# centreborelli/sat-bundleadjust

Hardware: AMD Instinct MI355X
Metric: LM iters/sec at 200 cams x 1M pts x 10M obs (affine, R+T) (higher is better)
Workload: dtype f64; 1 GPU; C4: 200 cams x 1000000 pts x 9998866 obs, affine, correction R+T, 1 fixed camera, seed 1; obs_per_rank0=9998866

## Files before the change

### sat-bundleadjust_amd/csrc/satba_capi.hip

```cpp
#include <hip/hip_runtime.h>

#include <algorithm>
#include <atomic>
#include <chrono>
#include <cmath>
#include <cstdarg>
#include <cstdio>
#include <cstdlib>
#include <cstring>
#include <new>
#include <string>
#include <thread>
#include <vector>

#include "../../include/satba.h"
#include "satba_chol.h"
#include "satba_kernels.h"
#include "satba_layout.h"
#include "satba_lm.h"
#include "satba_lmdev.h"
#include "satba_outliers.h"
#include "satba_triangulate.h"
#include "satba_tracks.h"
#include "satba_ftracks.h"
#include "satba_match.h"
#include "satba_rpcfit.h"
#include "satba_camapprox.h"
#include "satba_schur.h"
#include "satba_schur_items.h"

#include <dlfcn.h>

namespace {
struct Roctx {
    int (*push)(const char*) = nullptr;
    int (*pop)() = nullptr;
    Roctx() {
        for (const char* name : {"librocprofiler-sdk-roctx.so", "librocprofiler-sdk-roctx.so.1", "libroctx64.so", "libroctx64.so.4"}) {
            if (void* h = dlopen(name, RTLD_LAZY | RTLD_GLOBAL)) {
                push = reinterpret_cast<int (*)(const char*)>(dlsym(h, "roctxRangePushA"));
                pop = reinterpret_cast<int (*)()>(dlsym(h, "roctxRangePop"));
                if (push && pop) return;
                push = nullptr; pop = nullptr;
            }
        }
    }
};
inline const Roctx& roctx() { static const Roctx r; return r; }
struct Range {
    bool on;
    explicit Range(const char* name) : on(roctx().push != nullptr) { if (on) roctx().push(name); }
    ~Range() { if (on) roctx().pop(); }
};
}

using namespace satba;

static thread_local std::string g_err;

static int fail(int code, const char* fmt, ...) {
    char buf[512];
    va_list ap;
    va_start(ap, fmt);
    vsnprintf(buf, sizeof buf, fmt, ap);
    va_end(ap);
    g_err = buf;
    return code;
}

#define HIP_TRY(expr)                                                                                   \
    do {                                                                                                \
        hipError_t e_ = (expr);                                                                         \
        if (e_ != hipSuccess) return fail(SATBA_E_HIP, "%s: %s (%s:%d)", #expr, hipGetErrorString(e_), __FILE__, __LINE__); \
    } while (0)

constexpr int RED_SLOTS = 8, RED_MAX_GRID = 2048, RED_MAX_NV = 4;
struct SchurItems { int2* items = nullptr; SchurItem* desc = nullptr; int n_blocks = 0; };
static_assert(sizeof(SchurItemKey) == sizeof(int2) && offsetof(SchurItemKey, pair) == offsetof(int2, x) && offsetof(SchurItemKey, chunk) == offsetof(int2, y), "uploaded as int2");

struct satba_problem {
    int model = 0, M = 0, N = 0, NP = 0, c_p = 0, n_cam_fix = 0, n_pts_fix = 0, rank = 0, world = 1, f32 = 0, device = 0;
    long long K = 0, n_total = 0;
// ... 5 lines not shown
    int deterministic = 0;
    int split_env = -1;
    double *d_fx = nullptr, *d_bbox = nullptr, *d_fxcost = nullptr, *d_fxcost_new = nullptr, *d_fxcost0 = nullptr;
    int *d_fxflag = nullptr, *d_fxe = nullptr;
    bool fxcost_valid = false, fxcost_new_valid = false, fxcost0_valid = false;
    double w_max = 1.0, n_max_cam = 1.0, fx_shrink = 1.0;
    int fx_fallbacks = 0;
    bool scales_by_tail = false;
    bool gh_in_readers = false;
    bool q1_points_unformed = false;
    bool prep_fused = false;
    struct LmDev* d_lm = nullptr;
    struct LmSummary* h_lm = nullptr;
    struct LmSummary* h_lm_dev = nullptr;
    long long lm_ticks_queued = 0;
    hipStream_t own_stream = nullptr;
    double f_scale = 1.0, lead = 1.0;
    hipStream_t stream = nullptr;
    Layout L;
    int unit_weights = 0;
    double *d_cam_static = nullptr, *d_rpc = nullptr;
    double *d_x = nullptr, *d_xnew = nullptr, *d_camc = nullptr, *d_camc_new = nullptr;
    double *d_scale_inv = nullptr, *d_g = nullptr, *d_gh = nullptr, *d_gn = nullptr, *d_q1 = nullptr, *d_wv = nullptr;
    double *d_U = nullptr, *d_gc = nullptr, *d_V = nullptr, *d_PV = nullptr, *d_dc = nullptr, *d_dch = nullptr;
    double2 *d_f = nullptr, *d_ftmp = nullptr;
    bool f_valid = false;
    bool prof_lin = false;
    std::vector<hipEvent_t> prof_ev;
    size_t prof_used = 0;
    double* d_Jpm = nullptr;
    double *d_part = nullptr, *d_part3 = nullptr, *d_pair_part = nullptr;
    SchurItems items_chunked;
    SchurItems items_merged;
    double2* d_W = nullptr;
    SchurItems items_w;
    int lin_grid = 0, cm_chunks = 1, cm_chunks_w = 1;
    double* d_red = nullptr;
    unsigned* d_red_cnt = nullptr;
    double* d_stage = nullptr;
    size_t stage_len = 0;
    int* d_fail = nullptr;
    double* d_dinv = nullptr;
    CholWork chol;
    bool s_scaled = false;
    hipStream_t chol_stream = nullptr;
    hipEvent_t ev_fork = nullptr, ev_join = nullptr;
    int* d_arrive = nullptr;
    int* d_pair_cnt = nullptr;
    int* d_dg_cnt = nullptr;
    long long* d_ts = nullptr;
    int msg_epoch = 0;
    double* msg_packed = nullptr;
    bool beside_last = false;
    bool beside_off = false;
    int beside_clean = 0;
    int beside_retry_after = 64;
    int beside_timeouts = 0;
    double* d_scal = nullptr;
    double* d_keep = nullptr;
    double* d_lam_used = nullptr;
    bool prepared = false;
    double *d_xb_own = nullptr, *d_xb = nullptr;
    long long xb_len = 0;
    double* h_pin = nullptr;
    bool dir_global = false;
    double* d_dir_tab = nullptr;
    void* h_stage = nullptr;
    size_t h_stage_len = 0;
    struct CopyLane { char* pin = nullptr; hipEvent_t ev[2] = {nullptr, nullptr}; };
    CopyLane lanes[8];
    hipStream_t copy_stream = nullptr;
    bool lanes_ready = false;
    double* d_err_keep = nullptr;
    hipEvent_t ev_err = nullptr;
    double* d_x0 = nullptr;
    bool linearized = false, have_step = false;
    double create_ms[8] = {0, 0, 0, 0, 0, 0, 0, 0};
    std::vector<void*> allocs;

    double* payload() const { return d_xb + hdr; }
    RedBuf red(int slot) const { return RedBuf{d_red + (size_t)slot * RED_MAX_NV * RED_MAX_GRID, d_red_cnt + slot}; }
};
struct PhaseCtx {
    const int* gate = nullptr;
    const double *Delta_dev = nullptr, *coef_dev = nullptr, *lam_force_dev = nullptr, *sub_args_dev = nullptr;
    const int* first_dev = nullptr;
    int fuse_prep = -1;
    bool skip_lin_scales = false;
    bool decide1a_in_trial = false;
    bool decide2_in_trial = false;
};
struct FrontCtx {
    int arrive_epoch = 0;
    bool scale_in_finish = false;
    double lam = 0.0;
    const double* lam_dev = nullptr;
};
enum { RB_RES = 0, RB_LIN = 1, RB_PREP = 2, RB_JVP = 3, RB_BS = 4, RB_SUB = 5, RB_TRIAL = 6, RB_MISC = 7 };

template <class T>
static int dev_alloc(satba_problem* p, T** out, size_t count) {
    void* ptr = nullptr;
    HIP_TRY(hipMalloc(&ptr, (count ? count : 1) * sizeof(T)));
    p->allocs.push_back(ptr);
    *out = static_cast<T*>(ptr);
    return 0;
// ... 1321 lines not shown
}

int satba_get_layout(satba_problem* p, int32_t which, int64_t n, void* host_out) {
    if (!p || !host_out) return fail(SATBA_E_ARG, "null argument");
    const int64_t len = satba_layout_len(p, which);
    if (len < 0 || n != len) return fail(SATBA_E_ARG, "layout array %d has %lld entries, caller expects %lld", which, (long long)len, (long long)n);
    const Layout& L = p->L;
    const void* src = nullptr;
    size_t esz = sizeof(int);
    switch (which) {
        case SATBA_LAY_PERM: src = L.perm; break;
        case SATBA_LAY_RANK: src = L.rank; break;
        case SATBA_LAY_PT_CNT: src = L.pt_cnt; break;
        case SATBA_LAY_SLICE_BASE: src = L.slice_base; break;
        case SATBA_LAY_E_CAM: src = L.e_cam; break;
        case SATBA_LAY_OBS_POS: src = L.obs_pos; break;
        case SATBA_LAY_CM_PT: src = L.cm_pt; break;
        case SATBA_LAY_CM_POS: src = L.cm_pos; break;
        case SATBA_LAY_CM_IO: src = L.cm_io; break;
        case SATBA_LAY_IPT_OFS: src = L.ipt_ofs; break;
        case SATBA_LAY_CAM_OFS: src = L.cam_ofs; break;
        case SATBA_LAY_PAIR_OFS: src = L.pair_ofs; esz = sizeof(long long); break;
        case SATBA_LAY_PAIR_PTS: src = L.pair_pts; break;
        case SATBA_LAY_PAIR_PI: src = L.pair_pi; break;
        case SATBA_LAY_PAIR_PJ: src = L.pair_pj; break;
        case SATBA_LAY_PAIR_IJ: src = L.pair_ij; break;
        case SATBA_LAY_W_FIX: src = L.w_fix; break;
        case SATBA_LAY_SC_OFS: src = L.sc_ofs; break;
        case SATBA_LAY_PAIR_REC: src = L.pair_rec; break;
        case SATBA_LAY_PAIR_KK: src = L.pair_kk; break;
        case SATBA_LAY_CM_REC: src = L.cm_rec; break;
        case SATBA_LAY_CM_SC: src = L.cm_sc; break;
        case SATBA_LAY_DG_OFS: src = L.dg_ofs; break;
        default: return fail(SATBA_E_ARG, "unknown layout array %d", which);
    }
    HIP_TRY(hipSetDevice(p->device));
    HIP_TRY(hipStreamSynchronize(p->stream));
    if (len) HIP_TRY(hipMemcpy(host_out, src, esz * (size_t)len, hipMemcpyDeviceToHost));
    return 0;
}

int satba_get_info(const satba_problem* p, double* out, int32_t n) {
    if (!p || !out || n < 16) return fail(SATBA_E_ARG, "bad argument");
    for (int i = 0; i < n; ++i) out[i] = 0.0;
    for (int i = 0; i < 5; ++i) out[i] = p->create_ms[i];
    out[5] = p->L.P; out[6] = (double)p->L.E; out[7] = p->L.C; out[8] = p->unit_weights; out[9] = p->camc_lds; out[10] = p->rpc_lds;
    out[11] = p->cam_sums_lds; out[12] = p->deterministic; out[13] = p->cm_chunks; out[14] = p->lin_grid; out[15] = p->fx_fallbacks;
    if (n > 16) out[16] = (lm_device_loop_ok(p) && lm_device_loop_pays(p)) ? 1.0 : 0.0;
    if (n > 17) out[17] = p->beside_off ? -1.0 : (p->beside_last ? 1.0 : 0.0);
    if (n > 18) out[18] = p->beside_timeouts;
    if (n > 19) out[19] = p->L.wl_ready ? p->L.dg_spc : 0;
    if (n > 20) out[20] = slice_split(p);
    if (n > 21) out[21] = p->lin_rep_shift;
    return 0;
}

int satba_time_kernel(satba_problem* p, int32_t phase, int32_t reps, float* ms_avg) {
    if (!p || !ms_avg || reps <= 0) return fail(SATBA_E_ARG, "bad argument");
    if (phase < 0 || phase > 5) return fail(SATBA_E_ARG, "unknown phase %d", phase);
    if (phase >= 2 && !p->linearized) return fail(SATBA_E_STATE, "time_kernel: linearize first");
    HIP_TRY(hipSetDevice(p->device));
    hipEvent_t e0, e1;
    HIP_TRY(hipEventCreate(&e0));
    HIP_TRY(hipEventCreate(&e1));
    int rc = 0;
    auto once = [&]() -> int {
        switch (phase) {
            case 0: return launch_residual(p, false, p->d_f, p->d_scal);
            case 1: return launch_linearize_kernel(p, PhaseCtx{}, true);
            case 2: return launch_schur_kernel(p, nullptr, FrontCtx{}, schur_route(p, FrontCtx{}));
            case 3: {
                return dense_solve(p, nullptr, p->payload(), p->d_dch);
            }
            case 4: return launch_backsub_kernel(p, nullptr);
            default: return launch_jvp(p, nullptr, 1, p->d_q1, p->d_q1, p->d_scal, true);
        }
    };
    rc = once();
    if (!rc) {
        (void)hipEventRecord(e0, p->stream);
        for (int i = 0; i < reps && !rc; ++i) rc = once();
        (void)hipEventRecord(e1, p->stream);
        (void)hipEventSynchronize(e1);
        float ms = 0.f;
        (void)hipEventElapsedTime(&ms, e0, e1);
        *ms_avg = ms / reps;
    }
    (void)hipEventDestroy(e0);
    (void)hipEventDestroy(e1);
    p->linearized = false; p->have_step = false;
    return rc;
}

#include "satba_outliers_api.inc"
#include "satba_triangulate_api.inc"
#include "satba_rpcfit_api.inc"
#include "satba_camapprox_api.inc"
#include "satba_tracks_api.inc"
#include "satba_ftracks_api.inc"
#include "satba_match_api.inc"

}
```

### sat-bundleadjust_amd/csrc/satba_schur.h

```cpp
#pragma once
#include "satba_kernels.h"

namespace satba {

constexpr int PV_STRIDE = 16;
__device__ inline double schur_lambda(const double* __restrict__ hdr, double Delta, double lam_floor, double* __restrict__ keep, bool write) {
    const double gh_sq = hdr[SATBA_HDR_GH_SQ], jg_sq = hdr[SATBA_HDR_JG_SQ], xs_sq = hdr[SATBA_HDR_XS_SQ];
    if (!(Delta > 0.0)) {
        Delta = sqrt(xs_sq);
        if (Delta == 0.0) Delta = 1.0;
    }
    const double a = 0.5 * jg_sq, b = -gh_sq, ub = Delta / sqrt(gh_sq);
    double best = fmin(0.0, a * ub * ub + b * ub);
    if (a != 0.0) {
        const double ext = -0.5 * b / a;
        if (0.0 < ext && ext < ub) best = fmin(best, a * ext * ext + b * ext);
    }
    double lam = -best / (Delta * Delta);
    if (!(lam >= lam_floor)) lam = lam_floor;
    if (write) {
        keep[SATBA_KEEP_GINF] = fmax(keep[SATBA_KEEP_GINF], hdr[SATBA_HDR_GC_INF]);
        keep[SATBA_KEEP_GH_SQ] = gh_sq; keep[SATBA_KEEP_JG_SQ] = jg_sq; keep[SATBA_KEEP_XS_SQ] = xs_sq;
        keep[SATBA_KEEP_LAM] = lam;
        keep[SATBA_KEEP_DELTA] = Delta;
// ... 792 lines not shown
                    if constexpr (NP == 5) { acc[k++] += y0[r]; acc[k++] += y1[r]; }
                }
                if constexpr (NP == 5) { acc[k++] += e00; acc[k++] += e01; acc[k++] += e11; }
#pragma unroll
                for (int r = 0; r < 3; ++r) acc[k++] -= D[0][r] * b0 + D[1][r] * b1;
                if constexpr (NP == 5) { acc[k++] -= b0; acc[k++] -= b1; }
            } else {
                double Jc[2][NP], Jp[2][3];
                if constexpr (MODEL == RPC) {
                    ObsEval<MODEL, NP, true> e2;
                    e2.load_d(a, lst_sc[posc]);
                    rpc_jac_from_d<NP>(cc, r0.x, r0.y, r1.x, e2.Dr, Jc, Jp);
#pragma unroll
                    for (int k = 0; k < NP; ++k) { Jc[0][k] *= vm; Jc[1][k] *= vm; }
                    ux = uy = sx = sy = 1.0;
                } else {
                    double u, v;
                    project<MODEL, NP, true>(cc, nullptr, r0.x, r0.y, r1.x, false, u, v, Jc, Jp);
                    if (a.sc) { const double2 t = sc_now; ux = vm * t.x * t.x; uy = vm * t.y * t.y; }
                    sx = ux; sy = uy;
                }
                double A[2][3];
#pragma unroll
                for (int r = 0; r < 2; ++r) {
                    A[r][0] = Jp[r][0] * v00 + Jp[r][1] * v01 + Jp[r][2] * v02;
                    A[r][1] = Jp[r][0] * v01 + Jp[r][1] * v11 + Jp[r][2] * v12;
                    A[r][2] = Jp[r][0] * v02 + Jp[r][1] * v12 + Jp[r][2] * v22;
                }
                const double m00 = sx * ux * (A[0][0] * Jp[0][0] + A[0][1] * Jp[0][1] + A[0][2] * Jp[0][2]);
                const double m01 = sx * uy * (A[0][0] * Jp[1][0] + A[0][1] * Jp[1][1] + A[0][2] * Jp[1][2]);
                const double m11 = sy * uy * (A[1][0] * Jp[1][0] + A[1][1] * Jp[1][1] + A[1][2] * Jp[1][2]);
                const double ag0 = sx * (A[0][0] * r4.y + A[0][1] * r5.x + A[0][2] * r5.y);
                const double ag1 = sy * (A[1][0] * r4.y + A[1][1] * r5.x + A[1][2] * r5.y);
                int k = 0;
#pragma unroll
                for (int r = 0; r < NP; ++r) {
                    const double y0 = m00 * Jc[0][r] + m01 * Jc[1][r];
                    const double y1 = m01 * Jc[0][r] + m11 * Jc[1][r];
#pragma unroll
                    for (int q = r; q < NP; ++q) {
                        acc[k] -= Jc[0][q] * y0 + Jc[1][q] * y1;
                        acc[k] += ux * Jc[0][r] * Jc[0][q] + uy * Jc[1][r] * Jc[1][q];
                        ++k;
                    }
                }
#pragma unroll
                for (int r = 0; r < NP; ++r) acc[k++] -= Jc[0][r] * ag0 + Jc[1][r] * ag1;
            }
            __builtin_amdgcn_sched_barrier(0);
        }
    }
}

template <int MODEL, int NP>
__device__ __forceinline__ void schur_diag_body(const ObsArgs& a, const CamMajor& c, const SchurArgs& s, double* __restrict__ part, const int L, const int M,
                                                const int n_chunks, double2* s_coop, double (*s_red)[cam_acc_len(NP)]) {
    constexpr int CU = cam_acc_len(NP);
    int cam = L % M, chunk = L / M;
    if (s.diag_xcd) {
        const int x = L & 7, q = L >> 3;
        cam = q % M; chunk = (q / M) * 8 + x;
    }
    const int b = c.cam_ofs[cam], e = c.cam_ofs[cam + 1];
    const long long len = e - b;
    const int lo = b + (int)(len * chunk / n_chunks);
    const int hi = cam < a.n_cam_fix ? lo : b + (int)(len * (chunk + 1) / n_chunks);
    const int lane = threadIdx.x & 63, wave = threadIdx.x >> 6;
    double acc[CU];
#pragma unroll
    for (int k = 0; k < CU; ++k) acc[k] = 0.0;
    schur_diag_walk<MODEL, NP, LINC_THREADS>(a, s.PV, c.pt, c.io, s.wmode ? 1 : PV_STRIDE / 2, s.wmode ? s.zero_fix : (PV_STRIDE / 2) * a.N, cam, lo, hi,
                                             (int)threadIdx.x, s_coop + wave * (64 * 7), acc);
#pragma unroll
    for (int k = 0; k < CU; ++k) {
        const double t = wave_sum(acc[k]);
        if (lane == 0) s_red[wave][k] = t;
    }
    __syncthreads();
    if (threadIdx.x < CU) {
        double t = 0.0;
        for (int wv = 0; wv < LINC_THREADS / 64; ++wv) t += s_red[wv][threadIdx.x];
        part[((size_t)cam * n_chunks + chunk) * CU + threadIdx.x] = t;
    }
}
template <int MODEL, int NP>
__global__ __launch_bounds__(LINC_THREADS) void k_schur_diag(ObsArgs a, CamMajor c, SchurArgs s, double* __restrict__ part) {
    SATBA_GATE(a.gate);
    __shared__ double2 s_coop[(LINC_THREADS / 64) * 64 * 7];
    __shared__ double s_red[LINC_THREADS / 64][cam_acc_len(NP)];
    schur_diag_body<MODEL, NP>(a, c, s, part, (int)(blockIdx.y * gridDim.x + blockIdx.x), (int)gridDim.x, (int)gridDim.y, s_coop, s_red);
}
static_assert(LINC_THREADS == 256, "k_schur_both: both bodies run 256 threads");
template <int MODEL, int NP, bool UNITW>
__global__ __launch_bounds__(256) SATBA_PAIRS_WAVES_ATTR(MODEL, NP, UNITW) void k_schur_both(ObsArgs a, CamMajor c, SchurArgs s, double* __restrict__ part, double* __restrict__ S,
                                                                                      int n_diag, int n_diag_pad, int M, int n_chunks) {
    SATBA_GATE(a.gate);
    __shared__ double2 s_coop[4 * 64 * 7];
    __shared__ unsigned s_idx[4][3 * 64];
    __shared__ double s_red[4][cam_acc_len(NP)];
    if ((int)blockIdx.x < n_diag_pad) {
        if ((int)blockIdx.x < n_diag) schur_diag_body<MODEL, NP>(a, c, s, part, (int)blockIdx.x, M, n_chunks, s_coop, s_red);
        return;
    }
    schur_pairs_body<MODEL, NP, UNITW>(a, s, S, blockIdx.x - (unsigned)n_diag_pad, s_coop, s_idx);
}

__global__ __launch_bounds__(256) void k_schur_finish(int M, int NP, int n_c, int n_chunks, const double* __restrict__ part, double lam,
                                                      const double* __restrict__ lam_dev, double lead, const double* __restrict__ gc,
                                                      const double* __restrict__ scale_inv, double* __restrict__ S, double* __restrict__ rhs,
                                                      double* __restrict__ xb, int hdr_len, int nb_diag, int red_chunks,
                                                      const int2* __restrict__ pair_ij, const double* __restrict__ pair_part, const int* gate,
                                                      double* __restrict__ rhs_scaled = nullptr, int* __restrict__ clear = nullptr, int n_clear = 0) {
    SATBA_GATE(gate);
    if ((int)blockIdx.x >= nb_diag) {
        const long long n_pairs = (long long)M * (M - 1) / 2;
        const int NB2 = NP * NP;
        const long long idx = (long long)(blockIdx.x - nb_diag) * blockDim.x + threadIdx.x;
        if (idx >= n_pairs * NB2) return;
        const long long pair = idx / NB2;
        const int e = (int)(idx % NB2);
        double t = 0.0;
        int ch = 0;
        for (; ch + 4 <= red_chunks; ch += 4) {
            const double p0 = pair_part[((size_t)ch * n_pairs + pair) * NB2 + e], p1 = pair_part[((size_t)(ch + 1) * n_pairs + pair) * NB2 + e];
            const double p2 = pair_part[((size_t)(ch + 2) * n_pairs + pair) * NB2 + e], p3 = pair_part[((size_t)(ch + 3) * n_pairs + pair) * NB2 + e];
            t += p0; t += p1; t += p2; t += p3;
        }
        for (; ch < red_chunks; ++ch) t += pair_part[((size_t)ch * n_pairs + pair) * NB2 + e];
        const int2 ij = pair_ij[pair];
        const int r = e / NP, q = e % NP;
        if (rhs_scaled) t /= scale_inv[ij.y * NP + q] * scale_inv[ij.x * NP + r];
        S[(size_t)(ij.y * NP + q) + (size_t)(ij.x * NP + r) * n_c] = t;
        return;
    }
    if (lam_dev) lam = *lam_dev;
    const int CU = cam_acc_len(NP);
    const int gid = blockIdx.x * blockDim.x + threadIdx.x, idx = gid >> 3, sub = gid & 7;
    if (gid < hdr_len) xb[gid] = 0.0;
    if (gid < n_clear) clear[gid] = 0;
    if (n_chunks <= 0) return;
    const bool live = idx < M * CU;
    const int cam = live ? idx / CU : 0, k = live ? idx % CU : 0;
    const double t = schur_diag_total<false>(part, cam, n_chunks, CU, k, sub, live);
    if (!live || sub != 0) return;
    schur_diag_store<false>(cam, k, t, NP, n_c, lam, lead, gc, scale_inv, S, rhs, rhs_scaled);
}

}
```

### sat-bundleadjust_amd/csrc/satba_schur_api.inc

```
extern "C++" {
namespace {

int schur_items_build(satba_problem* p, SchurTable kind, SchurItems* t, long long dg_weight) {
    const bool w = kind == SCHUR_ITEMS_WEIGHTED;
    const std::vector<SchurItemKey> table = schur_item_order(kind, p->M, p->L.C, w ? p->L.dg_spc : 0, dg_weight);
    t->n_blocks = (int)(table.size() / 4);
    TRY(dev_alloc(p, &t->items, table.size()));
    HIP_TRY(hipMemcpy(t->items, table.data(), sizeof(int2) * table.size(), hipMemcpyHostToDevice));
    TRY(dev_alloc(p, &t->desc, table.size()));
    hipLaunchKernelGGL(k_schur_item_desc, dim3((unsigned)((table.size() + 255) / 256)), dim3(256), 0, p->stream, (long long)table.size(), t->items,
                       p->L.pair_ij, p->L.pair_ofs, p->L.C, t->desc, w ? p->L.dg_ofs : (const int*)nullptr, w ? p->L.n_dg : 1);
    HIP_TRY(hipGetLastError());
    return 0;
}
bool schur_merge_enough(const satba_problem* p) {
    const char* mg = getenv("SATBA_SCHUR_MERGE");
    return p->L.n_pairs >= 8192 || (mg && atoi(mg) != 0);
}
int schur_item_tables(satba_problem* p) {
    TRY(schur_items_build(p, SCHUR_ITEMS_CHUNKED, &p->items_chunked, 0));
    const char* mg = getenv("SATBA_SCHUR_MERGE");
    if (p->L.C > 1 && schur_merge_enough(p) && !(mg && atoi(mg) == 0)) TRY(schur_items_build(p, SCHUR_ITEMS_MERGED, &p->items_merged, 0));
    return 0;
}

struct SchurRoute {
    bool pairs_run, unit, weighted;
    const SchurItems* items;
    int n_chunks, red_chunks;
    bool dg_in_pairs, cm_rec;
    int dchunks, diag_xcd;
    bool both;
    bool finish_first, finish_direct, finish_scale;
    int finish_dchunks, finish_red_chunks, nb_diag;
    bool beside_ok;
    int wgs, arr_extra;
};

SchurRoute schur_route(const satba_problem* p, const FrontCtx& f) {
    const bool arrive = f.arrive_epoch != 0;
    static const bool one_launch = !(getenv("SATBA_SCHUR_ONE_LAUNCH") && atoi(getenv("SATBA_SCHUR_ONE_LAUNCH")) == 0);
    SchurRoute r;
    r.pairs_run = pairs_run(p); r.unit = unit_run(p); r.weighted = merged_records(p);
    const bool merged = r.pairs_run && r.unit && p->items_merged.desc;
    r.items = merged ? &p->items_merged : (r.weighted ? &p->items_w : &p->items_chunked);
    r.n_chunks = merged ? 1 : p->L.C; r.red_chunks = (r.pairs_run && p->L.C > 1 && !merged) ? p->L.C : 1;
    r.dg_in_pairs = r.weighted && r.pairs_run;
    r.dchunks = r.dg_in_pairs ? p->L.n_dg : (r.weighted ? p->cm_chunks_w : p->cm_chunks);
    r.diag_xcd = (!r.dg_in_pairs && r.dchunks % 8 == 0 && !getenv("SATBA_NO_DIAG_XCD")) ? 1 : 0;
    r.cm_rec = r.weighted && !r.dg_in_pairs;
    r.both = one_launch && !arrive && !r.dg_in_pairs && r.pairs_run;
    r.finish_first = arrive; r.finish_direct = arrive || (r.pairs_run && r.red_chunks == 1);
    r.finish_dchunks = (arrive && r.dg_in_pairs) ? 0 : r.dchunks; r.finish_red_chunks = arrive ? 1 : r.red_chunks;
    r.nb_diag = (int)((std::max<long long>(8ll * p->M * cam_acc_len(p->NP), p->hdr) + 255) / 256);
    r.finish_scale = f.scale_in_finish &&!r.finish_direct && 1 + CH_MAX_STEPS <= r.nb_diag * 256;
    const char* env = getenv("SATBA_CHOL_BESIDE");
    const bool items_ok = r.unit ? r.red_chunks == 1 : (schur_merge_enough(p) && p->model != RPC);
    r.beside_ok = !(env && atoi(env) == 0) && p->world == 1 && items_ok && r.pairs_run && p->n_c == p->M * p->NP && p->n_c > 128 && p->n_c <= 1024 &&
                  p->N > 0 && !p->beside_off;
    r.wgs = r.weighted ? 16 : 32; r.arr_extra = r.weighted ? 1 : 0;
    return r;
}

SchurArgs schur_args(const satba_problem* p, const FrontCtx& f, const SchurRoute& r, double* rhs) {
    SchurArgs s;
    s.PV = reinterpret_cast<const double2*>(p->d_PV);
    s.pair_ofs = p->L.pair_ofs; s.pair_pts = p->L.pair_pts; s.pair_pi = p->L.pair_pi; s.pair_pj = p->L.pair_pj;
    s.pair_ij = p->L.pair_ij; s.pair_part = p->d_pair_part; s.n_chunks = r.n_chunks; s.items = r.items->items; s.desc = r.items->desc; s.diag_xcd = r.diag_xcd;
    if (r.weighted) {
        s.PV = p->d_W; s.wmode = 1; s.zero_fix = p->L.zero_fix; s.n_dg = p->L.n_dg;
        s.pair_rec = p->L.pair_rec; s.pair_kk = p->L.pair_kk; s.cm_rec = p->L.cm_rec; s.cm_sc = p->L.cm_sc; s.dg_part = p->d_part3;
    }
    if (f.arrive_epoch) {
        s.arrive = p->d_arrive; s.arrive_epoch = f.arrive_epoch; s.pair_cnt = p->d_pair_cnt; s.fail = p->d_fail;
        if (r.dg_in_pairs) {
            s.dg_cnt = p->d_dg_cnt; s.dg_lam = f.lam; s.dg_lam_dev = f.lam_dev; s.dg_lead = p->lead; s.dg_gc = p->d_gc;
            s.dg_scale_inv = p->d_scale_inv; s.dg_rhs = rhs;
        }
    }
    return s;
}

template <int MODEL, int NP>
int launch_schur(satba_problem* p, const FrontCtx& f, const SchurRoute& r, const ObsArgs& a, double* S, double* rhs) {
    if (f.arrive_epoch && r.unit && r.red_chunks > 1) return fail(SATBA_E_STATE, "factorisation beside a unit-weight pair kernel with chunk partials");
    const CamMajor cm = cam_major(p, r.cm_rec);
    const SchurArgs s = schur_args(p, f, r, rhs);
    auto finish = [&]() {
        const long long outs = r.finish_red_chunks > 1 ? p->L.n_pairs * NP * NP : 0;
        hipLaunchKernelGGL(k_schur_finish, dim3((unsigned)(r.nb_diag + (outs + 255) / 256)), dim3(256), 0, p->stream, p->M, NP, p->n_c, r.finish_dchunks, p->d_part3,
                           f.lam, f.lam_dev, p->lead, p->d_gc, p->d_scale_inv, S, rhs, p->d_xb, (int)p->hdr, r.nb_diag, r.finish_red_chunks,
                           p->L.pair_ij, p->d_pair_part, a.gate, r.finish_scale ? p->d_dch : (double*)nullptr, r.finish_scale ? p->d_fail : (int*)nullptr,
                           r.finish_scale ? 1 + CH_MAX_STEPS : 0);
        p->s_scaled = r.finish_scale;
    };
    if (!r.dg_in_pairs && !r.both) hipLaunchKernelGGL((k_schur_diag<MODEL, NP>), dim3(p->M, r.dchunks), dim3(LINC_THREADS), 0, p->stream, a, cm, s, p->d_part3);
    if (r.finish_first) finish();
    if (r.pairs_run) {
        const dim3 igrid((unsigned)r.items->n_blocks);
        if (r.both) {
            const int n_diag = p->M * r.dchunks, n_diag_pad = (n_diag + 7) & ~7;
            const dim3 bgrid(igrid.x + (unsigned)n_diag_pad);
            if (r.unit) hipLaunchKernelGGL((k_schur_both<MODEL, NP, true>), bgrid, dim3(256), 0, p->stream, a, cm, s, p->d_part3, S, n_diag, n_diag_pad, p->M, r.dchunks);
            else hipLaunchKernelGGL((k_schur_both<MODEL, NP, false>), bgrid, dim3(256), 0, p->stream, a, cm, s, p->d_part3, S, n_diag, n_diag_pad, p->M, r.dchunks);
        }
        else if (r.unit) hipLaunchKernelGGL((k_schur_pairs<MODEL, NP, true>), igrid, dim3(256), 0, p->stream, a, s, S);
        else hipLaunchKernelGGL((k_schur_pairs<MODEL, NP, false>), igrid, dim3(256), 0, p->stream, a, s, S);
        HIP_TRY(hipGetLastError());
    }
    if (!r.finish_first) finish();
    HIP_TRY(hipGetLastError());
    return 0;
}

int schur_impl(satba_problem* p, const PhaseCtx& c, FrontCtx f, double lam, bool automatic, double Delta, double lam_floor) {
    Range range_("satba:schur");
    if (!p->linearized || (automatic && !p->prepared)) return fail(SATBA_E_STATE, automatic ? "schur_auto before prepare" : "schur before linearize");
    if (automatic) p->prepared = false;
    const SchurRoute r = schur_route(p, f);
    if (p->N > 0) {
        const bool w = r.weighted;
        hipLaunchKernelGGL(k_vinv, dim3((p->N + VINV_THREADS - 1) / VINV_THREADS), dim3(VINV_THREADS), 0, p->stream, p->N, lam, automatic ? p->d_xb : nullptr, Delta, lam_floor,
                           p->d_keep, p->d_V, p->d_scale_inv + p->n_c, p->d_lam_used, p->d_x + p->n_c, p->d_g + p->n_c, w ? reinterpret_cast<double*>(p->d_W) : p->d_PV,
                           p->L.perm, p->n_pts_fix, automatic ? c.Delta_dev : nullptr, automatic ? c.lam_force_dev : nullptr, c.gate,
                           w ? p->L.w_fix : (const int*)nullptr);
    } else if (automatic) {
        hipLaunchKernelGGL(k_lambda, dim3(1), dim3(1), 0, p->stream, p->d_xb, Delta, lam_floor, p->d_keep, c.Delta_dev, c.lam_force_dev, c.gate);
    }
    HIP_TRY(hipGetLastError());
    if (!r.pairs_run) HIP_TRY(hipMemsetAsync(p->d_xb + p->hdr, 0, sizeof(double) * ((size_t)p->n_c * p->n_c + p->n_c), p->stream));
    f.lam = lam; f.lam_dev = automatic ? p->d_keep + SATBA_KEEP_LAM : nullptr;
    return launch_schur_kernel(p, c.gate, f, r);
}

void beside_disable(satba_problem* p) {
    if (p->beside_timeouts > 0) p->beside_retry_after = std::min(p->beside_retry_after * 2, 1 << 20);
    p->beside_off = true; p->beside_clean = 0; ++p->beside_timeouts;
    (void)hipStreamSynchronize(p->chol_stream);
    (void)hipMemsetAsync(p->d_arrive, 0, sizeof(int) * (size_t)(p->M + 2) * SCHUR_ARRIVE_STRIDE, p->stream);
    (void)hipMemsetAsync(p->d_pair_cnt, 0, sizeof(int) * (size_t)std::max<long long>(p->L.n_pairs, 1), p->stream);
    (void)hipMemsetAsync(p->d_dg_cnt, 0, sizeof(int) * (size_t)p->M, p->stream);
}
bool beside_timed_out(satba_problem* p, const double* h) {
    if (!p->beside_last || !(h[SATBA_HDR_CHOL_FAIL] >= SATBA_CHOL_BESIDE_WAIT)) return false;
    beside_disable(p);
    return true;
}
int chol_front_streams(satba_problem* p) {
    if (p->chol_stream) return 0;
    int least = 0, greatest = 0, mine = 0;
    HIP_TRY(hipDeviceGetStreamPriorityRange(&least, &greatest));
    HIP_TRY(hipStreamGetPriority(p->stream, &mine));
    HIP_TRY(hipStreamCreateWithPriority(&p->chol_stream, hipStreamNonBlocking, mine != greatest ? greatest : least));
    HIP_TRY(hipEventCreateWithFlags(&p->ev_fork, hipEventDisableTiming));
    HIP_TRY(hipEventCreateWithFlags(&p->ev_join, hipEventDisableTiming));
    TRY(dev_alloc(p, &p->d_arrive, (size_t)(p->M + 2) * SCHUR_ARRIVE_STRIDE));
    HIP_TRY(hipMemsetAsync(p->d_arrive, 0, sizeof(int) * (size_t)(p->M + 2) * SCHUR_ARRIVE_STRIDE, p->stream));
    TRY(dev_alloc(p, &p->d_pair_cnt, (size_t)std::max<long long>(p->L.n_pairs, 1)));
    HIP_TRY(hipMemsetAsync(p->d_pair_cnt, 0, sizeof(int) * (size_t)std::max<long long>(p->L.n_pairs, 1), p->stream));
    TRY(dev_alloc(p, &p->d_dg_cnt, (size_t)p->M));
    HIP_TRY(hipMemsetAsync(p->d_dg_cnt, 0, sizeof(int) * (size_t)p->M, p->stream));
// ... 158 lines not shown
```

### sat-bundleadjust_amd/satba/engine_hip.py

```python
import ctypes as C
import os

import numpy as np

from .rpc_model import rpc_to_table
from .sharding import Shard

_LIB = None
LIB_PATH = os.environ.get("SATBA_LIB") or os.path.join(os.path.dirname(os.path.abspath(__file__)), "lib", "libsatba_hip.so")

CAM_MODELS = {"affine": 0, "perspective": 1, "rpc": 2}
LOSSES = {"linear": 0, "soft_l1": 1, "huber": 2, "cauchy": 3, "arctan": 4}
HDR_FIXED = 16

SYMBOLS = [
    "satba_last_error", "satba_version", "satba_problem_create", "satba_problem_destroy", "satba_set_stream",
    "satba_exchange_len", "satba_header_len", "satba_bind_exchange", "satba_configure", "satba_set_x", "satba_get_x",
    "satba_residuals", "satba_reprojection_errors", "satba_reprojection_errors_begin", "satba_reprojection_errors_fetch", "satba_linearize", "satba_prepare", "satba_schur", "satba_schur_auto", "satba_solve", "satba_subspace", "satba_subspace_products", "satba_trial", "satba_trial_gn",
    "satba_accept", "satba_camera_sums_fallback", "satba_read_header", "satba_get_blocks", "satba_get_jacobian", "satba_get_exchange",
    "satba_set_exchange", "satba_get_vector", "satba_time_kernel",
    "satba_packed_schur_len", "satba_pack_schur", "satba_solve_messages", "satba_solve_messages_bind", "satba_solve_messages_begin", "satba_solve_messages_arrived", "satba_solve_messages_end", "satba_unpack_schur",
    "satba_solve_lm", "satba_lm_step", "satba_lm_run", "satba_lm_state", "satba_lm_begin", "satba_lm_part", "satba_lm_poll", "satba_profile_linearize", "satba_profile_read", "satba_outliers", "satba_layout_len", "satba_get_layout", "satba_get_info",
    "satba_triangulate_pairwise", "satba_init_pts3d", "satba_init_pts3d_resident", "satba_snapshot_x",
    "satba_rpc_fit", "satba_rpc_localization", "satba_rpc_refit",
# ... 396 lines not shown
        out = np.zeros(17)
        _check(self.lib, self.lib.satba_lm_state(self._h, _ptr(out), 17))
        return dict(zip(self.LM_KEYS, out))

    def solve_lm(self, ftol=1e-8, xtol=1e-8, gtol=1e-8, max_nfev=None, loss="linear", f_scale=1.0, verbose=0):
        if loss not in LOSSES:
            raise ValueError("`loss` must be one of {}".format(list(LOSSES)))
        o = LmOpts(ftol=ftol, xtol=xtol, gtol=gtol, f_scale=f_scale, max_nfev=-1 if max_nfev is None else int(max_nfev),
                   loss=LOSSES[loss], verbose=int(verbose))
        st = LmStats()
        _check(self.lib, self.lib.satba_solve_lm(self._h, C.byref(o), C.byref(st)))
        return st

    def outliers(self, err=None, predef_thr=None, min_thr=1.0):
        check_predef_thr(predef_thr)
        thr = np.empty(self.n_cam)
        rm = np.zeros(max(self.n_obs, 1), dtype=np.uint8)
        n = C.c_int64()
        e = None if err is None else np.ascontiguousarray(err, dtype=np.float64)
        if e is not None and e.size != self.n_obs:
            raise ValueError("err has {} entries, expected {}".format(e.size, self.n_obs))
        _check(self.lib, self.lib.satba_outliers(self._h, _ptr(e) if e is not None else None, -1.0 if predef_thr is None else float(predef_thr),
                                                 float(min_thr), _ptr(thr), rm.ctypes.data_as(C.POINTER(C.c_uint8)), C.byref(n)))
        return thr, rm[: self.n_obs].astype(bool), int(n.value)

    def init_pts3d(self, camera_table, pairs, remove=None):
        tab = np.ascontiguousarray(camera_table, dtype=np.float64)
        if tab.shape[0] != self.n_cam:
            raise ValueError("camera table has {} rows, expected {}".format(tab.shape[0], self.n_cam))
        pr = np.ascontiguousarray(np.asarray(pairs, dtype=np.int32).reshape(-1, 2))
        rm = None
        if remove is not None:
            rm = np.ascontiguousarray(remove, dtype=np.uint8)
            if rm.size != self.n_obs:
                raise ValueError("remove has {} entries, expected {}".format(rm.size, self.n_obs))
        out = np.zeros((self.n_pts, 3), dtype=np.float32)
        n_tri = np.zeros(max(self.n_pts, 1), dtype=np.int32)
        ms = C.c_float(0.0)
        _check(self.lib, self.lib.satba_init_pts3d_resident(self._h, rm.ctypes.data_as(C.POINTER(C.c_uint8)) if rm is not None else None,
                                                            _ptr(tab), pr.shape[0], _ptr(pr, _ip), out.ctypes.data_as(C.POINTER(C.c_float)),
                                                            _ptr(n_tri, _ip), C.byref(ms)))
        return out, n_tri[: self.n_pts], ms.value

    def get_layout(self, name):
        which = LAYOUT[name]
        n = int(self.lib.satba_layout_len(self._h, which))
        if n < 0:
            raise ValueError("layout array {} does not exist (yet)".format(name))
        out = np.empty(n, dtype=np.int64 if name == "pair_ofs" else np.int32)
        _check(self.lib, self.lib.satba_get_layout(self._h, which, n, out.ctypes.data_as(C.c_void_p)))
        return out

    def info(self):
        v = np.zeros(22)
        _check(self.lib, self.lib.satba_get_info(self._h, _ptr(v), 22))
        keys = ["ms_uploads", "ms_sizes", "ms_ell", "ms_pairs", "ms_create", "ell_len", "pair_entries", "pair_chunks", "unit_weights",
                "camc_lds", "rpc_lds", "cam_sums_lds", "deterministic", "cm_chunks", "lin_grid", "fx_fallbacks", "device_loop", "chol_beside", "chol_beside_timeouts", "diag_items_per_chunk",
                "lanes_log2", "lin_rep_shift"]
        return dict(zip(keys, v[: len(keys)]))

    def get_blocks(self):
        U = np.empty((self.n_cam, self.n_p, self.n_p))
        gc = np.empty((self.n_cam, self.n_p))
        V = np.empty((self.n_pts, 6))
        gp = np.empty((self.n_pts, 3))
        _check(self.lib, self.lib.satba_get_blocks(self._h, _ptr(U), _ptr(gc), _ptr(V), _ptr(gp)))
        return U, gc, V, gp

    def get_jacobian(self):
        Jc = np.empty((self.n_obs, 2, self.n_p))
        Jp = np.empty((self.n_obs, 2, 3))
        _check(self.lib, self.lib.satba_get_jacobian(self._h, _ptr(Jc), _ptr(Jp)))
        return Jc, Jp

    def get_exchange(self, offset, n):
        out = np.empty(n)
        _check(self.lib, self.lib.satba_get_exchange(self._h, int(offset), int(n), _ptr(out)))
        return out

    def set_exchange(self, offset, values):
        values = np.ascontiguousarray(values, dtype=np.float64)
        _check(self.lib, self.lib.satba_set_exchange(self._h, int(offset), values.size, _ptr(values)))

    VECTORS = {"g": 0, "scale_inv": 1, "gn_h": 2, "q1": 3, "w": 4, "x_new": 5, "g_h": 6}

    def get_vector(self, name):
        out = np.empty(self.n)
        _check(self.lib, self.lib.satba_get_vector(self._h, self.VECTORS[name], _ptr(out)))
        return out

    KERNELS = {"residual": 0, "linearize": 1, "schur": 2, "cholesky": 3, "backsub": 4, "jvp": 5}

    def time_kernel(self, name, reps=10):
        ms = C.c_float()
        _check(self.lib, self.lib.satba_time_kernel(self._h, self.KERNELS[name], int(reps), C.byref(ms)))
        return ms.value
```

Measured before the change: 919.8 LM iters/sec.

## Split Schur diagonal so late cameras finish in-kernel behind pair work

Splits the Schur camera-diagonal accumulation at a camera index. Cameras before the split go through the existing diag kernel and finish step. The trailing cameras (about 3/16 of the tile columns) are accumulated inside the pairs kernel, or in a separate late kernel. The last chunk for each camera reduces the partials, writes the diagonal block and signals per-camera arrival for the beside-running Cholesky. The aim is to let the factorisation start on early columns while the tail diagonal work overlaps pair computation. The cost is extra atomics, counter resets and the risk of ordering bugs.

After: 933.9 LM iters/sec, median of 6. 1.5% higher.

```diff
diff --git a/sat-bundleadjust_amd/csrc/satba_capi.hip b/sat-bundleadjust_amd/csrc/satba_capi.hip
--- a/sat-bundleadjust_amd/csrc/satba_capi.hip
+++ b/sat-bundleadjust_amd/csrc/satba_capi.hip
@@ -28,6 +28,7 @@
 #include "satba_camapprox.h"
 #include "satba_schur.h"
 #include "satba_schur_items.h"
+#include "satba_diag_split.h"
 
 #include <dlfcn.h>
 
@@ -139,6 +140,7 @@
     int msg_epoch = 0;
     double* msg_packed = nullptr;
     bool beside_last = false;
+    int diag_split_last = -1;
     bool beside_off = false;
     int beside_clean = 0;
     int beside_retry_after = 64;
@@ -1566,6 +1568,7 @@
     if (n > 19) out[19] = p->L.wl_ready ? p->L.dg_spc : 0;
     if (n > 20) out[20] = slice_split(p);
     if (n > 21) out[21] = p->lin_rep_shift;
+    if (n > 22) out[22] = p->diag_split_last;
     return 0;
 }
 
diff --git a/sat-bundleadjust_amd/csrc/satba_diag_split.h b/sat-bundleadjust_amd/csrc/satba_diag_split.h
--- /dev/null
+++ b/sat-bundleadjust_amd/csrc/satba_diag_split.h
@@ -0,0 +1,18 @@
+#pragma once
+
+namespace satba {
+inline int diag_split_tiles(int M, int NP) { return (M * NP + 63) / 64; }
+inline int diag_split_camera(int M, int NP, int late_cols, bool applies = true) {
+    if (!applies || late_cols <= 0 || M <= 0 || NP <= 0) return M;
+    const int T = diag_split_tiles(M, NP);
+    if (late_cols >= T) return 0;
+    const int c = 64 * (T - late_cols) / NP;
+    return c < M ? c : M;
+}
+inline int diag_split_forced(int M, int from, bool applies = true) {
+    if (!applies) return M;
+    return from < 0 ? 0 : (from > M ? M : from);
+}
+inline int diag_late_cols_default(int T) { return 3 * T / 16; }
+constexpr bool DIAG_LATE_TAIL_DEFAULT = true;
+}
diff --git a/sat-bundleadjust_amd/csrc/satba_schur.h b/sat-bundleadjust_amd/csrc/satba_schur.h
--- a/sat-bundleadjust_amd/csrc/satba_schur.h
+++ b/sat-bundleadjust_amd/csrc/satba_schur.h
@@ -868,15 +868,10 @@
     }
 }
 
-template <int MODEL, int NP>
-__device__ __forceinline__ void schur_diag_body(const ObsArgs& a, const CamMajor& c, const SchurArgs& s, double* __restrict__ part, const int L, const int M,
-                                                const int n_chunks, double2* s_coop, double (*s_red)[cam_acc_len(NP)]) {
+template <int MODEL, int NP, bool PUBLISH>
+__device__ __forceinline__ void schur_diag_chunk(const ObsArgs& a, const CamMajor& c, const SchurArgs& s, double* __restrict__ part, const int cam, const int chunk,
+                                                 const int n_chunks, double2* s_coop, double (*s_red)[cam_acc_len(NP)]) {
     constexpr int CU = cam_acc_len(NP);
-    int cam = L % M, chunk = L / M;
-    if (s.diag_xcd) {
-        const int x = L & 7, q = L >> 3;
-        cam = q % M; chunk = (q / M) * 8 + x;
-    }
     const int b = c.cam_ofs[cam], e = c.cam_ofs[cam + 1];
     const long long len = e - b;
     const int lo = b + (int)(len * chunk / n_chunks);
@@ -896,8 +891,47 @@
     if (threadIdx.x < CU) {
         double t = 0.0;
         for (int wv = 0; wv < LINC_THREADS / 64; ++wv) t += s_red[wv][threadIdx.x];
-        part[((size_t)cam * n_chunks + chunk) * CU + threadIdx.x] = t;
-    }
+        double* const out = part + ((size_t)cam * n_chunks + chunk) * CU + threadIdx.x;
+        if constexpr (PUBLISH) __hip_atomic_store(out, t, __ATOMIC_RELAXED, __HIP_MEMORY_SCOPE_AGENT);
+        else *out = t;
+    }
+}
+template <int MODEL, int NP>
+__device__ __forceinline__ void schur_diag_body(const ObsArgs& a, const CamMajor& c, const SchurArgs& s, double* __restrict__ part, const int L, const int M,
+                                                const int n_chunks, double2* s_coop, double (*s_red)[cam_acc_len(NP)]) {
+    int cam = L % M, chunk = L / M;
+    if (s.diag_xcd) {
+        const int x = L & 7, q = L >> 3;
+        cam = q % M; chunk = (q / M) * 8 + x;
+    }
+    schur_diag_chunk<MODEL, NP, false>(a, c, s, part, cam, chunk, n_chunks, s_coop, s_red);
+}
+template <int MODEL, int NP>
+__device__ __forceinline__ void schur_diag_late_body(const ObsArgs& a, const CamMajor& c, const SchurArgs& s, double* __restrict__ part, double* __restrict__ S,
+                                                     const int L, const int cam0, const int n_chunks, double2* s_coop, double (*s_red)[cam_acc_len(NP)]) {
+    constexpr int CU = cam_acc_len(NP);
+    const int cam = cam0 + L / n_chunks, chunk = L % n_chunks;
+    schur_diag_chunk<MODEL, NP, true>(a, c, s, part, cam, chunk, n_chunks, s_coop, s_red);
+    __shared__ int s_last;
+    asm volatile("s_waitcnt vmcnt(0)" ::: "memory");
+    __syncthreads();
+    if (threadIdx.x == 0) {
+        const int old = __hip_atomic_fetch_add(s.dg_cnt + cam, 1, __ATOMIC_RELAXED, __HIP_MEMORY_SCOPE_AGENT);
+        s_last = (old == n_chunks - 1) ? 1 : 0;
+        if (s_last) __hip_atomic_store(s.dg_cnt + cam, 0, __ATOMIC_RELAXED, __HIP_MEMORY_SCOPE_AGENT);
+    }
+    __syncthreads();
+    if (!s_last) return;
+    const double lam = s.dg_lam_dev ? *s.dg_lam_dev : s.dg_lam;
+    for (int o0 = 0; o0 < CU; o0 += LINC_THREADS / 8) {
+        const int k = o0 + ((int)threadIdx.x >> 3), sub = (int)threadIdx.x & 7;
+        const bool live = k < CU;
+        const double t = schur_diag_total<true>(part, cam, n_chunks, CU, live ? k : 0, sub, live);
+        if (live && sub == 0) schur_diag_store<true>(cam, k, t, NP, a.n_c, lam, s.dg_lead, s.dg_gc, s.dg_scale_inv, S, s.dg_rhs, nullptr);
+    }
+    asm volatile("s_waitcnt vmcnt(0)" ::: "memory");
+    __syncthreads();
+    if (threadIdx.x == 0) __hip_atomic_fetch_add(s.arrive + (size_t)SCHUR_ARRIVE_STRIDE * cam, 1, __ATOMIC_RELAXED, __HIP_MEMORY_SCOPE_AGENT);
 }
 template <int MODEL, int NP>
 __global__ __launch_bounds__(LINC_THREADS) void k_schur_diag(ObsArgs a, CamMajor c, SchurArgs s, double* __restrict__ part) {
@@ -920,13 +954,34 @@
     }
     schur_pairs_body<MODEL, NP, UNITW>(a, s, S, blockIdx.x - (unsigned)n_diag_pad, s_coop, s_idx);
 }
+template <int MODEL, int NP>
+__global__ __launch_bounds__(LINC_THREADS) void k_schur_diag_late(ObsArgs a, CamMajor c, SchurArgs s, double* __restrict__ part, double* __restrict__ S, int cam0, int n_chunks) {
+    SATBA_GATE(a.gate);
+    __shared__ double2 s_coop[(LINC_THREADS / 64) * 64 * 7];
+    __shared__ double s_red[LINC_THREADS / 64][cam_acc_len(NP)];
+    schur_diag_late_body<MODEL, NP>(a, c, s, part, S, (int)blockIdx.x, cam0, n_chunks, s_coop, s_red);
+}
+template <int MODEL, int NP>
+__global__ __launch_bounds__(256) SATBA_PAIRS_WAVES_ATTR(MODEL, NP, true) void k_schur_pairs_diag_late(ObsArgs a, CamMajor c, SchurArgs s, double* __restrict__ part,
+                                                                                                   double* __restrict__ S, int n_pair_wgs, int n_pair_pad, int cam0, int n_chunks) {
+    SATBA_GATE(a.gate);
+    __shared__ double2 s_coop[4 * 64 * 7];
+    __shared__ unsigned s_idx[4][3 * 64];
+    __shared__ double s_red[4][cam_acc_len(NP)];
+    if ((int)blockIdx.x < n_pair_pad) {
+        if ((int)blockIdx.x < n_pair_wgs) schur_pairs_body<MODEL, NP, true>(a, s, S, blockIdx.x, s_coop, s_idx);
+        return;
+    }
+    schur_diag_late_body<MODEL, NP>(a, c, s, part, S, (int)blockIdx.x - n_pair_pad, cam0, n_chunks, s_coop, s_red);
+}
 
 __global__ __launch_bounds__(256) void k_schur_finish(int M, int NP, int n_c, int n_chunks, const double* __restrict__ part, double lam,
                                                       const double* __restrict__ lam_dev, double lead, const double* __restrict__ gc,
                                                       const double* __restrict__ scale_inv, double* __restrict__ S, double* __restrict__ rhs,
                                                       double* __restrict__ xb, int hdr_len, int nb_diag, int red_chunks,
                                                       const int2* __restrict__ pair_ij, const double* __restrict__ pair_part, const int* gate,
-                                                      double* __restrict__ rhs_scaled = nullptr, int* __restrict__ clear = nullptr, int n_clear = 0) {
+                                                      double* __restrict__ rhs_scaled = nullptr, int* __restrict__ clear = nullptr, int n_clear = 0,
+                                                      int cam_hi = -1, int* __restrict__ arrive = nullptr) {
     SATBA_GATE(gate);
     if ((int)blockIdx.x >= nb_diag) {
         const long long n_pairs = (long long)M * (M - 1) / 2;
@@ -954,8 +1009,9 @@
     const int gid = blockIdx.x * blockDim.x + threadIdx.x, idx = gid >> 3, sub = gid & 7;
     if (gid < hdr_len) xb[gid] = 0.0;
     if (gid < n_clear) clear[gid] = 0;
+    if (arrive && gid < cam_hi) __hip_atomic_fetch_add(arrive + (size_t)SCHUR_ARRIVE_STRIDE * gid, 1, __ATOMIC_RELAXED, __HIP_MEMORY_SCOPE_AGENT);
     if (n_chunks <= 0) return;
-    const bool live = idx < M * CU;
+    const bool live = idx < (cam_hi >= 0 ? cam_hi : M) * CU;
     const int cam = live ? idx / CU : 0, k = live ? idx % CU : 0;
     const double t = schur_diag_total<false>(part, cam, n_chunks, CU, k, sub, live);
     if (!live || sub != 0) return;
diff --git a/sat-bundleadjust_amd/csrc/satba_schur_api.inc b/sat-bundleadjust_amd/csrc/satba_schur_api.inc
--- a/sat-bundleadjust_amd/csrc/satba_schur_api.inc
+++ b/sat-bundleadjust_amd/csrc/satba_schur_api.inc
@@ -35,6 +35,8 @@
     int finish_dchunks, finish_red_chunks, nb_diag;
     bool beside_ok;
     int wgs, arr_extra;
+    int c_split;
+    bool late_tail;
 };
 
 SchurRoute schur_route(const satba_problem* p, const FrontCtx& f) {
@@ -58,7 +60,12 @@
     const bool items_ok = r.unit ? r.red_chunks == 1 : (schur_merge_enough(p) && p->model != RPC);
     r.beside_ok = !(env && atoi(env) == 0) && p->world == 1 && items_ok && r.pairs_run && p->n_c == p->M * p->NP && p->n_c > 128 && p->n_c <= 1024 &&
                   p->N > 0 && !p->beside_off;
-    r.wgs = r.weighted ? 16 : 32; r.arr_extra = r.weighted ? 1 : 0;
+    const bool split_applies = r.beside_ok && r.unit && !r.dg_in_pairs && r.red_chunks == 1;
+    const char *lf = getenv("SATBA_DIAG_LATE_FROM"), *lc = getenv("SATBA_DIAG_LATE_COLS"), *lp = getenv("SATBA_DIAG_LATE_PLACE");
+    r.c_split = (lf && *lf) ? diag_split_forced(p->M, atoi(lf), split_applies)
+                            : diag_split_camera(p->M, p->NP, (lc && *lc) ? atoi(lc) : diag_late_cols_default(diag_split_tiles(p->M, p->NP)), split_applies);
+    r.late_tail = (lp && *lp) ? (*lp == 'b' || *lp == 'B') : DIAG_LATE_TAIL_DEFAULT;
+    r.wgs = r.weighted ? 16 : 32; r.arr_extra = (r.weighted || r.c_split < p->M) ? 1 : 0;
     return r;
 }
 
@@ -73,7 +80,7 @@
     }
     if (f.arrive_epoch) {
         s.arrive = p->d_arrive; s.arrive_epoch = f.arrive_epoch; s.pair_cnt = p->d_pair_cnt; s.fail = p->d_fail;
-        if (r.dg_in_pairs) {
+        if (r.dg_in_pairs || r.c_split < p->M) {
             s.dg_cnt = p->d_dg_cnt; s.dg_lam = f.lam; s.dg_lam_dev = f.lam_dev; s.dg_lead = p->lead; s.dg_gc = p->d_gc;
             s.dg_scale_inv = p->d_scale_inv; s.dg_rhs = rhs;
         }
@@ -86,15 +93,19 @@
     if (f.arrive_epoch && r.unit && r.red_chunks > 1) return fail(SATBA_E_STATE, "factorisation beside a unit-weight pair kernel with chunk partials");
     const CamMajor cm = cam_major(p, r.cm_rec);
     const SchurArgs s = schur_args(p, f, r, rhs);
+    const int c_split = f.arrive_epoch ? r.c_split : p->M;
+    const bool late = c_split < p->M;
+    p->diag_split_last = c_split;
     auto finish = [&]() {
         const long long outs = r.finish_red_chunks > 1 ? p->L.n_pairs * NP * NP : 0;
         hipLaunchKernelGGL(k_schur_finish, dim3((unsigned)(r.nb_diag + (outs + 255) / 256)), dim3(256), 0, p->stream, p->M, NP, p->n_c, r.finish_dchunks, p->d_part3,
                            f.lam, f.lam_dev, p->lead, p->d_gc, p->d_scale_inv, S, rhs, p->d_xb, (int)p->hdr, r.nb_diag, r.finish_red_chunks,
                            p->L.pair_ij, p->d_pair_part, a.gate, r.finish_scale ? p->d_dch : (double*)nullptr, r.finish_scale ? p->d_fail : (int*)nullptr,
-                           r.finish_scale ? 1 + CH_MAX_STEPS : 0);
+                           r.finish_scale ? 1 + CH_MAX_STEPS : 0, late ? c_split : -1, late ? p->d_arrive : (int*)nullptr);
         p->s_scaled = r.finish_scale;
     };
-    if (!r.dg_in_pairs && !r.both) hipLaunchKernelGGL((k_schur_diag<MODEL, NP>), dim3(p->M, r.dchunks), dim3(LINC_THREADS), 0, p->stream, a, cm, s, p->d_part3);
+    if (!r.dg_in_pairs && !r.both && c_split > 0)
+        hipLaunchKernelGGL((k_schur_diag<MODEL, NP>), dim3(c_split, r.dchunks), dim3(LINC_THREADS), 0, p->stream, a, cm, s, p->d_part3);
     if (r.finish_first) finish();
     if (r.pairs_run) {
         const dim3 igrid((unsigned)r.items->n_blocks);
@@ -104,9 +115,17 @@
             if (r.unit) hipLaunchKernelGGL((k_schur_both<MODEL, NP, true>), bgrid, dim3(256), 0, p->stream, a, cm, s, p->d_part3, S, n_diag, n_diag_pad, p->M, r.dchunks);
             else hipLaunchKernelGGL((k_schur_both<MODEL, NP, false>), bgrid, dim3(256), 0, p->stream, a, cm, s, p->d_part3, S, n_diag, n_diag_pad, p->M, r.dchunks);
         }
+        else if (late && r.late_tail) {
+            const int n_pad = ((int)igrid.x + 7) & ~7;
+            hipLaunchKernelGGL((k_schur_pairs_diag_late<MODEL, NP>), dim3((unsigned)(n_pad + (p->M - c_split) * r.dchunks)), dim3(256), 0, p->stream, a, cm, s, p->d_part3, S,
+                               (int)igrid.x, n_pad, c_split, r.dchunks);
+        }
         else if (r.unit) hipLaunchKernelGGL((k_schur_pairs<MODEL, NP, true>), igrid, dim3(256), 0, p->stream, a, s, S);
         else hipLaunchKernelGGL((k_schur_pairs<MODEL, NP, false>), igrid, dim3(256), 0, p->stream, a, s, S);
         HIP_TRY(hipGetLastError());
+        if (late && !r.late_tail)
+            hipLaunchKernelGGL((k_schur_diag_late<MODEL, NP>), dim3((unsigned)((p->M - c_split) * r.dchunks)), dim3(LINC_THREADS), 0, p->stream, a, cm, s, p->d_part3, S,
+                               c_split, r.dchunks);
     }
     if (!r.finish_first) finish();
     HIP_TRY(hipGetLastError());
diff --git a/sat-bundleadjust_amd/satba/engine_hip.py b/sat-bundleadjust_amd/satba/engine_hip.py
--- a/sat-bundleadjust_amd/satba/engine_hip.py
+++ b/sat-bundleadjust_amd/satba/engine_hip.py
@@ -472,11 +472,11 @@
         return out
 
     def info(self):
-        v = np.zeros(22)
-        _check(self.lib, self.lib.satba_get_info(self._h, _ptr(v), 22))
+        v = np.zeros(23)
+        _check(self.lib, self.lib.satba_get_info(self._h, _ptr(v), 23))
         keys = ["ms_uploads", "ms_sizes", "ms_ell", "ms_pairs", "ms_create", "ell_len", "pair_entries", "pair_chunks", "unit_weights",
                 "camc_lds", "rpc_lds", "cam_sums_lds", "deterministic", "cm_chunks", "lin_grid", "fx_fallbacks", "device_loop", "chol_beside", "chol_beside_timeouts", "diag_items_per_chunk",
-                "lanes_log2", "lin_rep_shift"]
+                "lanes_log2", "lin_rep_shift", "diag_late_from"]
         return dict(zip(keys, v[: len(keys)]))
 
     def get_blocks(self):
```
